# JayKickliter/Multirate.jl

Hardware: AMD Instinct MI355X
Metric: Msamples/s in (Float32, 147//160, 24*147 taps) + achieved HBM GB/s vs roofline (higher is better)
Workload: dtype f32

## Files before the change

multirate.jl_amd/csrc/mrhip_internal.h:

```cpp
#pragma once

#include <hip/hip_runtime.h>
#include <hip/hip_ext.h>

#include <cstdint>
#include <cstdlib>
#include <string>
#include <vector>

#include "multirate_hip.h"

namespace mrhip {

void set_error(const std::string &msg);
int fail(int code, const std::string &msg);

#define MRHIP_CHECK_HIP(expr)                                                                  \
    do {                                                                                       \
        hipError_t _e = (expr);                                                                \
        if (_e != hipSuccess)                                                                  \
            return ::mrhip::fail(MRHIP_ERR_HIP, std::string(#expr) + ": " + hipGetErrorString(_e)); \
    } while (0)

inline bool dtype_is_complex(int dt) { return dt == MRHIP_C64 || dt == MRHIP_C128; }
inline bool dtype_is_f64(int dt) { return dt == MRHIP_F64 || dt == MRHIP_C128; }
inline size_t dtype_scalar_size(int dt) { return dtype_is_f64(dt) ? 8 : 4; }
inline size_t dtype_size(int dt) { return dtype_scalar_size(dt) * (dtype_is_complex(dt) ? 2 : 1); }

int64_t taps2pfb(const void *h, int64_t hLen, int th, int64_t Nphi, void *out);
int64_t nextphase(int64_t phase, int64_t L, int64_t M);
int64_t outputlength_ratio(int64_t inputlength, int64_t L, int64_t M, int64_t initialPhi);
int64_t inputlength_ratio(int64_t outputlength, int64_t L, int64_t M, int64_t initialPhi);

struct CallPlan {
    int64_t n_out = 0;
    int64_t phi0 = 1, d0 = 1;
    int64_t phi_end = 1;
    int64_t d_end = 1;
    bool short_input = false;
};
CallPlan plan_rational(int kind, int64_t L, int64_t M, int64_t phiIdx, int64_t inputDeficit, int64_t xLen);

struct ArbState {
    double acc = 1.0;
    int64_t phiIdx = 1;
    double alpha = 0.0;
    int64_t xIdx = 1;
    int64_t inputDeficit = 1;
};
int64_t run_arbitrary_schedule(ArbState &st, double delta, int64_t Nphi, int64_t xLen,
                               std::vector<int32_t> *n_idx, std::vector<double> *acc_out, int mod_form = 0);
int64_t run_arbitrary_schedule_piece(ArbState &st, double delta, int64_t Nphi, int64_t xLen, int32_t *n_idx, double *acc_out,
                                     int64_t max_outputs, bool *done, int mod_form = 0);

constexpr int kSchedSeg = 64;
constexpr int kSchedGroup = 64 * kSchedSeg;
constexpr int kSchedMaxWin = 64;
constexpr int kSchedNoFail = 0x7fffffff;
constexpr int kSchedSpanSizes = 5;
constexpr int kSchedSpanBase = 64;
inline int sched_span_index(long long tile_out) { int z = 0; while (z + 1 < kSchedSpanSizes && (static_cast<long long>(kSchedSpanBase) << z) < tile_out) ++z; return z; }

struct SchedPlan {
    double delta, N, invN;
    double umin, inv_umin;
    double G, inv_G;
    double halfwin;
    int ncand, nwin;
    int pow2;
    int ok;
};
struct SchedPieceState {
    double acc;
    long long xIdx;
    double drift;
    double ksteps;
};
struct SchedStatus {
    int fail_piece;
    int done;
    long long end_k;
    double end_acc;
    long long end_xIdx;
    int max_span[kSchedSpanSizes];
    int groups_done;
    int pad[2];
    long long x_len;
    double end_drift;
    double end_ksteps;
};
struct SchedGroupEntry { double shift; int advance; int next; };
struct SchedGroupStart { double shift; long long advance; int cand; int pad; };
struct SchedPieceArgs {
    SchedPieceState *state;
    SchedStatus *status;
    double *pathT;
    int *pathW;
    SchedGroupEntry *gtab;
    SchedGroupStart *gstart;
    int *sched_n;
    double *sched_acc;
    long long k0;
    long long x_len;
    int piece, ngroups;
    int corrupt_group;
};
SchedPlan make_sched_plan(double delta, int64_t Nphi, int win_mult = 1, int win_min = 4);
struct SchedFuseArgs;
hipError_t launch_schedule_piece(const SchedPlan &c, const SchedPieceArgs &a, hipStream_t s, const SchedFuseArgs *fu = nullptr);
struct DevStream;
struct DevCall;
struct SchedBeginArgs {
    DevStream *rec;
    SchedStatus *status;
    SchedPieceState *state;
    int use_host;
    double acc; long long xIdx; double drift, ksteps;
    const DevCall *x_from;
};
struct SchedFinishArgs {
    DevStream *rec, *mirror;
    DevCall *call;
    SchedStatus *status;
    SchedPieceState *state;
    SchedPieceState *fail_state;
    int *sched_n; double *sched_acc;
    long long *count_out;
    long long k_first;
    double ks_first;
    long long pmax, est, x_len, y_capacity;
    int np;
    int serial_fallback;
};
struct SchedFuseArgs {
    int begin, finish;
    int fold_chain;
    SchedBeginArgs b;
    long long b_x_len, b_k_first;
    SchedFinishArgs f;
};
hipError_t launch_sched_begin(const SchedBeginArgs &a, long long x_len, long long k_first, hipStream_t s);
hipError_t launch_sched_finish(const SchedPlan &c, const SchedFinishArgs &a, hipStream_t s);
__host__ __device__ inline long long sched_piece_steps(double ks, long long pmax)
{
    long long P = kSchedGroup;
    while (P * 2 <= pmax && static_cast<double>(P * 2) <= 16.0 * ks) P *= 2;
    return P;
}
double sched_anchor_host(const SchedPlan &c, double acc_p, double k);

struct DevStream {
    long long phiIdx, inputDeficit;
    double acc;
    double drift, ksteps;
    long long per_pos;
    long long n_written;
    long long calls;
    long long fallback_steps;
    int error;
    int sched_fail;
};
struct DevCall {
    long long n_out;
    long long u0, d0;
    unsigned steps_per_channel, total_steps, spc_magic, pad0;
    long long per_pos, per_xbase;
    long long k_done;
    long long x_len;
};
__host__ __device__ inline unsigned step_magic(long long spc)
{
    return spc <= 1 ? 0xffffffffu : static_cast<unsigned>((1ULL << 32) / static_cast<unsigned long long>(spc));
}
struct CallPlanPOD { long long n_out, phi0, d0, phi_end, d_end; int short_input; };
__host__ __device__ inline CallPlanPOD plan_rational_pod(int kind, long long L, long long M, long long phiIdx, long long inputDeficit, long long xLen)
{
    CallPlanPOD p{0, 1, 1, 1, 1, 0};
    if (kind == MRHIP_FIR_STANDARD) { p.n_out = xLen; return p; }
    if (kind == MRHIP_FIR_INTERPOLATOR) { p.n_out = L * xLen; return p; }
    p.phi0 = kind == MRHIP_FIR_DECIMATOR ? 1 : phiIdx;
    p.d0 = inputDeficit;
    if (xLen < inputDeficit) { p.short_input = 1; p.n_out = 0; p.phi_end = phiIdx; p.d_end = inputDeficit - xLen; return p; }
    const long long a = (xLen - inputDeficit + 1) * L - p.phi0 + 1;
    p.n_out = a >= 0 ? (a + M - 1) / M : -((-a) / M);
    const long long u_end = (p.phi0 - 1) + p.n_out * M;
    p.phi_end = u_end % L + 1;
    p.d_end = p.d0 + u_end / L - xLen;
    return p;
}

struct PolyArgs {
    const void *x;
    void *y;
    const void *hist;
    void *hist_new;
    const void *taps;
    long long x_stride, y_stride;
    long long x_len;
    long long n_out;
    long long u0;
    long long d0;
    long long zero_start_below;
    int L, M, T, H;
    int nch;
    DevStream *rec;
    const DevCall *dyn;
    long long phi_end, d_end;
    const struct MultiDesc *multi;
    int multi_n;
    struct RingDev *ring_dev;
    struct RingHost *ring_host;
};

struct MultiDesc {
    const void *x;
    void *y;
    const void *hist;
    void *hist_new;
    const void *taps;
    DevStream *rec;
    long long x_stride, y_stride, x_len, n_out, u0, d0, phi_end, d_end;
    unsigned steps_per_channel, total_steps, spc_magic;
    int nch;
    int P_blk, q0;
};

constexpr int kRingDepth = 64;
constexpr int kRingTraceRows = 512, kRingTraceTiles = 32;
constexpr int kRingShards = 32;
struct RingDesc {
    unsigned long long x, y;
    long long x_stride, y_stride, x_len, n_out;
    long long u0, d0;
    unsigned long long tile_base;
    unsigned ngrabs, seq_lo;
    unsigned steps_per_channel, total_steps;
    unsigned spc_magic, flags;
    unsigned long long seq;
    unsigned long long pad[3];
};
static_assert(sizeof(RingDesc) == 128, "RingDesc is 16 quad-words");
constexpr int kRingKeyQword = 8;
struct RingHost {
    unsigned long long head;
    unsigned long long close;
    unsigned long long stopped;
    unsigned long long arrived, grid;
    unsigned long long pad[3];
    unsigned long long done[kRingDepth];
    RingDesc desc[kRingDepth];
};
struct RingDev {
    unsigned long long head;
    unsigned long long closed;
    unsigned long long idle_ticks;
    unsigned long long opts;
    unsigned long long pad[4];
    unsigned long long hist_seq[kRingDepth];
    unsigned chunk_done[kRingDepth];
    unsigned shard_done[kRingDepth][kRingShards][32];
    unsigned long long stats[24];
    unsigned long long arrived;
    unsigned long long grid;
    unsigned long long flush_req;
    unsigned long long flush_pub;
    unsigned long long flush_pad[12];
    unsigned long long flush_ent[kRingDepth][2];
    unsigned long long flush_claim[8][16];
    unsigned long long flush_done[8][16];
    unsigned long long next_ticket[8][16];
    __attribute__((aligned(128))) RingDesc desc[kRingDepth];
    unsigned long long trace[kRingTraceRows][3 * kRingTraceTiles];
};

struct ShiftFold {
    void *hist_new;
    unsigned *done;
};

struct ArbArgs {
    const void *x;
    void *y;
    const void *hist;
    const void *taps;
    const void *dtaps;
    const int *n_idx;
    const double *acc;
    long long x_stride, y_stride;
    long long x_len;
    long long n_out;
    int T, H, Nphi;
    int nch;
    const DevCall *dyn;
    ShiftFold fold;
};

struct FarrowArgs {
    const void *x;
    void *y;
    const void *hist;
    const double *pnfb;
    const int *n_idx;
    const double *acc;
    long long x_stride, y_stride;
    long long x_len;
    long long n_out;
    int T, H, polyorder;
    int tap_f32;
    int nch;
    int seam_below;
    const DevCall *dyn;
    ShiftFold fold;
};

struct HistArgs {
    const void *x;
    const void *hist_old;
    void *hist_new;
    long long x_stride;
    long long x_len;
    int H;
    int nch;
    const DevCall *dyn;
};

struct TileArgs {
    int c;
    int P;
    int J;
    int tile_len;
    int copyB_offset_bytes;
    int stage_bytes;
    int dma_rounds;
    int ablate;
    int x_aligned16;
    int by_position;
    long long tiles_per_channel;
    long long total_tiles;
};

struct PairArgs {
    int c;
    int P;
    int cM;
    int J;
    int tile_len;
    int tail;
    int dma_rounds;
    int stage_bytes;
    int ns;
    int nc;
    int x_f64, r_f64;
    int ablate;
    unsigned steps_per_channel;
    unsigned total_steps;
    unsigned steps_per_group;
    int ngroups;
    int grid_cap;
    int flags_off;
    int pad_every;
    int bank_off;
    int static_grabs;
    int rt;
    int rt_rd;
    unsigned *counters;
    unsigned spc_magic;
    int Sout, lds_step, run_chunks, q0;
    unsigned run_magic;
    long long o0;
    long long tile_in;
    long long tile_out;
    long long tiles_per_channel;
    long long total_tiles;
    unsigned long long *probe;
};

constexpr size_t kCounterBytes = 33 * 256;

struct ArbTileArgs {
    int cpl;
    int tap_pitch;
    int bank_elems;
    int x_offset_bytes;
    int max_span;
    int prefetch;
    int copyb_pad;
    int pipe;
    int row_pitch;
    int dma_slots;
    long long tile_out;
    long long tiles_per_channel;
    long long total_tiles;
    unsigned *counters;
    int run_tiles;
};

__device__ __forceinline__ void tiles_take_dyn(long long &n_out, ArbTileArgs &ta, long long &ngroups, const DevCall *dyn)
{
    ngroups = ta.tiles_per_channel > 0 ? ta.total_tiles / ta.tiles_per_channel : 1;
    if (dyn) {
        n_out = dyn->n_out;
        ta.tiles_per_channel = (n_out + ta.tile_out - 1) / ta.tile_out;
        ta.total_tiles = ta.tiles_per_channel * ngroups;
    }
}

struct LaunchEvents { hipEvent_t start = nullptr, stop = nullptr; };
extern thread_local LaunchEvents g_launch_events;

template <typename F, typename... Args>
inline void launch_kernel(F kfn, dim3 grid, dim3 block, size_t lds, hipStream_t s, Args... args)
{
    const LaunchEvents ev = g_launch_events;
    g_launch_events = LaunchEvents{};
    if (ev.start && ev.stop)
        hipExtLaunchKernelGGL(kfn, grid, block, static_cast<std::uint32_t>(lds), s, ev.start, ev.stop, 0u, args...);
    else
        hipLaunchKernelGGL(kfn, grid, block, lds, s, args...);
}

hipError_t occupancy_cached(const void *kfn, unsigned block, size_t lds, int *per_cu);

inline int env_int_read(const char *name, int dflt)
{
    const char *v = std::getenv(name);
    return v && *v ? std::atoi(v) : dflt;
}
inline bool env_dynamic()
{
    static const bool d = env_int_read("MRHIP_ENV_DYNAMIC", 0) != 0;
    return d;
}
#define MRHIP_ENV_INT(name, dflt) ([]() -> int { static const int v_ = ::mrhip::env_int_read(name, dflt); \
                                                 return ::mrhip::env_dynamic() ? ::mrhip::env_int_read(name, dflt) : v_; }())

struct TypeKey {
    bool x_f64;
    bool r_f64;
    bool complex_x;
};

hipError_t launch_poly_generic(const TypeKey &tk, bool fused, const PolyArgs &a, hipStream_t s, const char **kname);
hipError_t launch_arb_generic(const TypeKey &tk, bool fused, const ArbArgs &a, hipStream_t s, const char **kname);
hipError_t launch_farrow(const TypeKey &tk, bool fused, const FarrowArgs &a, hipStream_t s, const char **kname);
bool plan_farrow_tiled(const TypeKey &tk, const FarrowArgs &a, const int32_t *n_idx_host, const int *spans, int num_cus, ArbTileArgs *out, size_t *lds);
hipError_t launch_farrow_tiled(const TypeKey &tk, bool fused, const FarrowArgs &a, const ArbTileArgs &ta, size_t lds, hipStream_t s,
                               const char **kname, int num_cus);
hipError_t launch_shiftin(const TypeKey &tk, const HistArgs &a, hipStream_t s);
bool polyfit_rows(const double *y, int64_t n, int polyorder, double *coef);
bool plan_rational_opair(const TypeKey &tk, bool fused, const PolyArgs &a, int num_cus, PairArgs *out, dim3 *block, size_t *lds, int force_wgpc = 0);
bool plan_rational_opair_blocks(const TypeKey &tk, bool fused, const PolyArgs &a, int num_cus, PairArgs *out, dim3 *block, size_t *lds, int *nblocks);
hipError_t launch_rational_opair(bool fused, const PolyArgs &a, const PairArgs &pa, dim3 block, size_t lds, hipStream_t s,
                                 const char **kname, int num_cus, unsigned *counters);
constexpr bool opair_instantiated(bool fused, int smin, int T) { return !fused || (smin <= 1 && T % 4 == 0); }
bool plan_fir_stream(const TypeKey &tk, const PolyArgs &a, int num_cus, PairArgs *out, dim3 *block, size_t *lds);
hipError_t launch_fir_stream(bool fused, const PolyArgs &a, const PairArgs &pa, dim3 block, size_t lds, hipStream_t s,
                             const char **kname, int num_cus, unsigned *counters);
bool plan_arb_tiled(const TypeKey &tk, const ArbArgs &a, const int32_t *n_idx_host, const int *spans, int num_cus, ArbTileArgs *out, size_t *lds);
bool plan_arb_pipe(const TypeKey &tk, const ArbArgs &a, long long span256, ArbTileArgs *out, size_t *lds);
hipError_t launch_arb_pipe(const TypeKey &tk, bool fused, const ArbArgs &a, const ArbTileArgs &ta, size_t lds, hipStream_t s,
                           const char **kname, int num_cus);
struct ArbLaneArgs {
    int ring;
    int pitch8;
    int stretch;
    int chunk_max;
    int ngroups;
    int y16;
    unsigned *counters;
};
bool arb_lane_eligible(const TypeKey &tk, int T, int H, int64_t nch, double rate, int64_t x_len, int64_t x_stride, int64_t y_stride);
bool plan_arb_lane(const TypeKey &tk, const ArbArgs &a, double rate, ArbLaneArgs *out, size_t *lds);
hipError_t launch_arb_lane(bool fused, const ArbArgs &a, const ArbLaneArgs &la, size_t lds, hipStream_t s, const char **kname, int num_cus);
hipError_t launch_arb_tiled(const TypeKey &tk, bool fused, const ArbArgs &a, const ArbTileArgs &ta, size_t lds, hipStream_t s,
                            const char **kname, int num_cus);
bool plan_poly_tiled(const TypeKey &tk, const PolyArgs &a, int num_cus, ArbTileArgs *out, size_t *lds);
hipError_t launch_poly_tiled(const TypeKey &tk, bool fused, const PolyArgs &a, const ArbTileArgs &ta, size_t lds, hipStream_t s,
                             const char **kname, int num_cus);
bool plan_phase_stationary(const TypeKey &tk, const PolyArgs &a, int num_cus, TileArgs *out, dim3 *grid, dim3 *block,
                           size_t *lds);
hipError_t launch_poly_phase_stationary(const TypeKey &tk, bool fused, const PolyArgs &a, const TileArgs &ta, dim3 grid,
                                        dim3 block, size_t lds, hipStream_t s, const char **kname, int num_cus);

}
```

multirate.jl_amd/csrc/opair_kernel.inc:

```
#include <algorithm>
#include <cstdio>
#include <cstdlib>
#include <type_traits>
#include <vector>

#include "mrhip_internal.h"
#include "pair_device.h"
#include "pair_loader.h"

#pragma clang fp contract(off)

#ifndef MRHIP_OPAIR_WIDE_LONG
#define MRHIP_OPAIR_WIDE_LONG 1
#endif

namespace mrhip {
namespace {

constexpr int kOMaxThreads = 512;
constexpr int kOGroups = 32;

#define opair_env_int(name, dflt) MRHIP_ENV_INT(name, dflt)

using namespace dev;

__device__ __forceinline__ float fma_r(float a, float b, float c) { return __builtin_fmaf(a, b, c); }
__device__ __forceinline__ double fma_r(double a, double b, double c) { return __builtin_fma(a, b, c); }

template <bool FUSED, bool FIRST, bool COND, typename R>
__device__ __forceinline__ R slot_mac(R tap, R w, R acc, bool used)
{
    if constexpr (FIRST) {
        const R p = tap * w;
        if constexpr (COND) return used ? p : static_cast<R>(-0.0);
        else return p;
    } else if constexpr (FUSED) {
        const R r = fma_r(tap, w, acc);
        if constexpr (COND) return used ? r : acc;
        else return r;
    } else {
        R p = tap * w;
        if constexpr (COND) p = used ? p : static_cast<R>(-0.0);
        return acc + p;
    }
}

template <int T, bool FUSED, int NC, int SMIN, typename TXS, typename R, int MODE = 0>
#ifndef MRHIP_OPAIR_WIDE_WAVES
#define MRHIP_OPAIR_WIDE_WAVES 3
#endif
#ifndef MRHIP_RING_WAVES
#define MRHIP_RING_WAVES 4
#endif
__global__ __launch_bounds__(sizeof(R) == 8 && T > 32 ? kOMaxThreads : kOMaxThreads + 64, sizeof(R) == 8 ? (T > 32 ? 2 : MRHIP_OPAIR_WIDE_WAVES) : (MODE == 2 ? MRHIP_RING_WAVES : 3))
void rational_opair_kernel(PolyArgs a, PairArgs pa)
{
    constexpr unsigned ES = static_cast<unsigned>(sizeof(TXS)) * NC;
    constexpr unsigned OS = static_cast<unsigned>(sizeof(R)) * NC;
    constexpr int NW = static_cast<int>(ES / 4);
    static_assert(NW == 1 || NW == 2 || NW == 4, "sample size");
    using pair_t = std::conditional_t<NW == 1, v2u_t, v4u_t>;
    constexpr int SPRD = NW == 4 ? 1 : 2;
    constexpr int W = T + SMIN + 2;
    constexpr int NPR = (W + SPRD - 1) / SPRD;
    constexpr int NA = T + 1, NB = T + 2;

    extern __shared__ __attribute__((aligned(16))) unsigned char smem[];
    const unsigned lds_base = static_cast<unsigned>(reinterpret_cast<uintptr_t>(smem));
    const int tid = threadIdx.x;
    const int wave = __builtin_amdgcn_readfirstlane(tid >> 6), lane = tid & 63;
    const int ncw = (blockDim.x >> 6) - 1;
    constexpr bool RING = MODE == 2;
    if constexpr (MODE == 0) pair_take_dyn(a, pa);

    if (wave == ncw) {
        if constexpr (RING) pair_ring_loader_wave<NW, static_cast<int>(OS)>(a, pa, smem, lane);
        else pair_loader_wave<NW, MODE != 1>(a, pa, smem, lane);
        return;
    }
    if constexpr (RING) { if (blockIdx.x == 0) return; }
    volatile unsigned *const tile_flag = reinterpret_cast<volatile unsigned *>(smem + pa.flags_off);

    const int Li = static_cast<int>(a.L), Mi = static_cast<int>(a.M);
    int u0 = static_cast<int>(a.u0);
    const bool act = 2 * tid + 1 < pa.P;
    int uA = u0 + (act ? 2 * tid : 0) * Mi, uB = uA + Mi;
    int qA = uA / Li, phA = uA - qA * Li;
    int qB = uB / Li, phB = uB - qB * Li;
    int run0 = qA & ~1;
    int offA = qA - run0;
    int dB = qB - run0 - SMIN;
    R tapA[NA], tapB[NB];
    auto gather_taps = [&]() {
        const R *__restrict__ ca = static_cast<const R *>(a.taps) + static_cast<long long>(phA) * T;
        const R *__restrict__ cb = static_cast<const R *>(a.taps) + static_cast<long long>(phB) * T;
        R colA[T], colB[T];
#pragma unroll
        for (int i = 0; i < T; ++i) { colA[i] = ca[i]; colB[i] = cb[i]; }
#pragma unroll
        for (int j = 0; j < NA; ++j) {
            const R t0 = j < T ? colA[j] : R(0), t1 = j >= 1 ? colA[j - 1] : R(0);
            tapA[j] = act ? (offA == 0 ? t0 : t1) : R(0);
        }
#pragma unroll
        for (int j = 0; j < NB; ++j) {
            const R t0 = j < T ? colB[j] : R(0), t1 = (j >= 1 && j - 1 < T) ? colB[j - 1] : R(0), t2 = j >= 2 ? colB[j - 2] : R(0);
            tapB[j] = act ? (dB == 0 ? t0 : dB == 1 ? t1 : t2) : R(0);
        }
    };
    if constexpr (RING) {
#pragma unroll
        for (int j = 0; j < NA; ++j) tapA[j] = R(0);
#pragma unroll
        for (int j = 0; j < NB; ++j) tapB[j] = R(0);
        u0 = -1;
    } else if (pa.bank_off >= 0) {
        constexpr int PT = (T + 4) | 1;
        R *const bank = reinterpret_cast<R *>(smem + pa.bank_off);
        const R *__restrict__ tg = static_cast<const R *>(a.taps);
        const int ntaps = Li * T;
        for (int idx = tid; idx < ntaps; idx += ncw * 64) {
            const int col = idx / T, i = idx - col * T;
            bank[col * PT + 2 + i] = tg[idx];
        }
        asm volatile("s_waitcnt vmcnt(0) lgkmcnt(0)" ::: "memory");
        __builtin_amdgcn_s_barrier();
        const R *ba = bank + (act ? phA : 0) * PT + 2 - offA;
        const R *bb = bank + (act ? phB : 0) * PT + 2 - (act ? dB : 0);
#pragma unroll
        for (int j = 0; j < NA; ++j) tapA[j] = ba[j];
#pragma unroll
        for (int j = 0; j < NB; ++j) tapB[j] = bb[j];
#pragma unroll
        for (int j = 0; j < NA; ++j) pin(tapA[j]);
#pragma unroll
        for (int j = 0; j < NB; ++j) pin(tapB[j]);
    } else {
        const R *__restrict__ ca = static_cast<const R *>(a.taps) + static_cast<long long>(phA) * T;
        const R *__restrict__ cb = static_cast<const R *>(a.taps) + static_cast<long long>(phB) * T;
        R colA[T], colB[T];
#pragma unroll
        for (int i = 0; i < T; ++i) { colA[i] = ca[i]; colB[i] = cb[i]; }
#pragma unroll
        for (int j = 0; j < NA; ++j) {
            const R t0 = j < T ? colA[j] : R(0), t1 = j >= 1 ? colA[j - 1] : R(0);
            tapA[j] = act ? (offA == 0 ? t0 : t1) : R(0);
        }
#pragma unroll
        for (int j = 0; j < NB; ++j) {
            const R t0 = j < T ? colB[j] : R(0), t1 = (j >= 1 && j - 1 < T) ? colB[j - 1] : R(0), t2 = j >= 2 ? colB[j - 2] : R(0);
            tapB[j] = act ? (dB == 0 ? t0 : dB == 1 ? t1 : t2) : R(0);
        }
    }
    bool useA0 = offA == 0, useAT = offA == 1;
    bool useB0 = dB == 0, useB1 = dB <= 1, useBT = dB >= 1, useBT1 = dB == 2;

    const int n_out = static_cast<int>(a.n_out);
#ifdef MRHIP_OPAIR_PROBE
    unsigned long long pr_wait = 0, pr_tiles = 0;
    const unsigned long long pr_t0 = clock64(), pr_w0 = wall_clock64();
#endif
    unsigned ring_opts = 0;
    if constexpr (RING) ring_opts = static_cast<unsigned>(__builtin_amdgcn_readfirstlane(static_cast<int>(ld_sc1(&a.ring_dev->opts))));
    unsigned long long rs_bar = 0, rs_drain = 0;
    const unsigned long long rs_t0 = RING ? wall_clock64() : 0ull;
    bool pend = false;
    int p_stage = 0;
    unsigned p_slot = 0, p_shard = 0, p_cnt = 0, p_nshards = 0, p_seq_lo = 0, p_seq_hi = 0;
    for (int s = 0;; s = (s + 1 == pa.ns ? 0 : s + 1)) {
#ifdef MRHIP_OPAIR_PROBE
        const unsigned long long pr_a = clock64();
#endif
        unsigned long long rs_b0 = 0;
        if constexpr (RING) { if (ring_opts & 256u) rs_b0 = wall_clock64(); }
        __builtin_amdgcn_s_barrier();
        asm volatile("" ::: "memory");
        if constexpr (RING) { if (ring_opts & 256u) rs_bar += wall_clock64() - rs_b0; }
#ifdef MRHIP_OPAIR_PROBE
        pr_wait += clock64() - pr_a;
        ++pr_tiles;
#endif
        int J, remaining;
        R *__restrict__ yc;
        unsigned ring_flags = 0, ring_slot = 0, ring_shard = 0, ring_cnt = 0, ring_nshards = 0, ring_seq_lo = 0, ring_seq_hi = 0;
        if constexpr (RING) {
            auto word = [&](int w) -> unsigned { return static_cast<unsigned>(__builtin_amdgcn_readfirstlane(static_cast<int>(tile_flag[kRingTileWords * s + w]))); };
            const unsigned tj = word(0);
            ring_flags = word(1);
            if (pend) {
                pend = false;
                const unsigned long long rs_d0 = (ring_opts & 256u) ? wall_clock64() : 0ull;
                if (!(ring_opts & 16u)) vm_drain();
                if (ring_opts & 256u) rs_drain += wall_clock64() - rs_d0;
                if (lane == 0) {
                    unsigned *const wg_done = reinterpret_cast<unsigned *>(smem + pa.flags_off) + kRingTileWords * pa.ns;
                    const unsigned prev = __hip_atomic_fetch_add(wg_done + p_stage, 1u, __ATOMIC_RELAXED, __HIP_MEMORY_SCOPE_WORKGROUP);
                    if (prev + 1u == static_cast<unsigned>(ncw)) {
                        __hip_atomic_store(wg_done + p_stage, 0u, __ATOMIC_RELAXED, __HIP_MEMORY_SCOPE_WORKGROUP);
                        ring_grab_done(a.ring_dev, a.ring_host, p_slot, (static_cast<unsigned long long>(p_seq_hi) << 32) | p_seq_lo, p_shard, p_cnt, p_nshards);
                    }
                }
            }
            if (tj == 0u) break;
            if (ring_flags & 2u) continue;
            J = static_cast<int>(tj);
            yc = reinterpret_cast<R *>((static_cast<unsigned long long>(word(3)) << 32) | word(2));
            remaining = static_cast<int>(word(4));
            const int u0_t = static_cast<int>(word(5));
            ring_slot = word(6); ring_shard = word(7); ring_seq_lo = word(8); ring_seq_hi = word(9); ring_cnt = word(10); ring_nshards = word(11);
            if (u0_t != u0) {
                u0 = u0_t;
                uA = u0 + (act ? 2 * tid : 0) * Mi; uB = uA + Mi;
                qA = uA / Li; phA = uA - qA * Li;
                qB = uB / Li; phB = uB - qB * Li;
                run0 = qA & ~1; offA = qA - run0; dB = qB - run0 - SMIN;
                gather_taps();
                useA0 = offA == 0; useAT = offA == 1;
                useB0 = dB == 0; useB1 = dB <= 1; useBT = dB >= 1; useBT1 = dB == 2;
            }
        } else {
            const unsigned tg = static_cast<unsigned>(__builtin_amdgcn_readfirstlane(static_cast<int>(tile_flag[2 * s])));
            const unsigned tj = static_cast<unsigned>(__builtin_amdgcn_readfirstlane(static_cast<int>(tile_flag[2 * s + 1])));
            if (tj == 0u) break;
            const TileAt ta = pair_tile_at(pa, tg, tj);
            J = ta.jt;
            yc = static_cast<R *>(a.y) + (static_cast<long long>(ta.ch) * a.y_stride + static_cast<long long>(ta.st) * pa.Sout) * NC;
            remaining = n_out - ta.st * pa.Sout;
        }
        const bool full = remaining >= (J - 1) * pa.Sout + pa.P;
        unsigned lane_t;
        asm volatile("v_mbcnt_lo_u32_b32 %0, -1, 0\n\tv_mbcnt_hi_u32_b32 %0, -1, %0" : "=v"(lane_t));
        const unsigned tid_t = static_cast<unsigned>(wave) * 64u + lane_t;
        const unsigned my_out = 2u * tid_t;
        const unsigned uA_t = static_cast<unsigned>(u0) + (2u * tid_t < static_cast<unsigned>(pa.P) ? 2u * tid_t : 0u) * static_cast<unsigned>(Mi);
        const unsigned R_t = (uA_t / static_cast<unsigned>(Li)) & ~1u;
        const unsigned wbase = lds_base + static_cast<unsigned>(s) * pa.stage_bytes + (R_t - static_cast<unsigned>(pa.q0)) * ES;

        auto run_steps = [&](auto full_tag) {
            constexpr bool FULL = decltype(full_tag)::value;
            constexpr int KP = NPR < (NW == 1 ? 5 : 3) ? NPR : (NW == 1 ? 5 : 3);
            constexpr int NPRV = (NPR + KP - 1) / KP * KP;
            constexpr bool PAIRED_WAITS = KP >= 5;
            pair_t pring[KP];
            char *const ybytes = reinterpret_cast<char *>(yc);
            auto read_pair = [&](auto off_tag, unsigned addr) -> pair_t {
                constexpr int OFFP = decltype(off_tag)::value;
                if constexpr (NW == 1) return lds_read_b64<OFFP * 8>(addr);
                else return lds_read_b128<OFFP * 16>(addr);
            };
            static_for<0, KP>([&](auto I) { pring[decltype(I)::value] = read_pair(I, wbase); });
#pragma unroll 1
            for (int j = 0; j < J; ++j) {
                const int jn = j + 1 < J ? j + 1 : j;
                const unsigned wcur = wbase + static_cast<unsigned>(j) * pa.lds_step * ES;
                const unsigned wnext = wbase + static_cast<unsigned>(jn) * pa.lds_step * ES;
                R accA[NC] = {}, accB[NC] = {};
                static_for<0, NPRV>([&](auto I) {
                    constexpr int r = decltype(I)::value;
                    constexpr int slot = r % KP;
                    if constexpr (r < NPR) {
                        if constexpr (!PAIRED_WAITS) lgkm_wait<ring_younger(r, NPR, KP, 0)>(pring[slot]);
                        else if constexpr (r % 2 == 0) {
                            if constexpr (r + 1 < NPR) lgkm_wait2<ring_younger_pair(r, NPR, KP, 0)>(pring[slot], pring[(r + 1) % KP]);
                            else lgkm_wait<ring_younger(r, NPR, KP, 0)>(pring[slot]);
                        }
                        R wv[2][NC];
                        if constexpr (NW == 4) {
                            wv[0][0] = __hiloint2double(static_cast<int>(pring[slot].y), static_cast<int>(pring[slot].x));
                            wv[0][1] = __hiloint2double(static_cast<int>(pring[slot].w), static_cast<int>(pring[slot].z));
                        } else if constexpr (sizeof(TXS) == 8) {
                            wv[0][0] = __hiloint2double(static_cast<int>(pring[slot].y), static_cast<int>(pring[slot].x));
                            wv[1][0] = __hiloint2double(static_cast<int>(pring[slot].w), static_cast<int>(pring[slot].z));
                        } else if constexpr (NC == 1) {
                            wv[0][0] = static_cast<R>(__uint_as_float(pring[slot].x)); wv[1][0] = static_cast<R>(__uint_as_float(pring[slot].y));
                        } else {
                            wv[0][0] = static_cast<R>(__uint_as_float(pring[slot].x)); wv[0][1] = static_cast<R>(__uint_as_float(pring[slot].y));
                            wv[1][0] = static_cast<R>(__uint_as_float(pring[slot].z)); wv[1][1] = static_cast<R>(__uint_as_float(pring[slot].w));
                        }
                        static_for<0, SPRD>([&](auto H) {
                            constexpr int js = SPRD * r + decltype(H)::value;
                            constexpr int jb = js - SMIN;
                            constexpr bool a_lo = js < 1, a_hi = js > T - 1;
                            constexpr bool b_lo = jb < 2, b_hi = jb > T - 1;
#pragma unroll
                            for (int cc = 0; cc < NC; ++cc) {
                                const R w = wv[decltype(H)::value][cc];
                                if constexpr (js < NA) {
                                    const bool used = (a_lo ? useA0 : true) && (a_hi ? useAT : true);
                                    accA[cc] = slot_mac<FUSED, js == 0, a_lo || a_hi, R>(tapA[js], w, accA[cc], used);
                                }
                                if constexpr (jb >= 0 && jb < NB) {
                                    const bool used = (b_lo ? (jb == 0 ? useB0 : useB1) : true) && (b_hi ? (jb == T ? useBT : useBT1) : true);
                                    accB[cc] = slot_mac<FUSED, jb == 0, b_lo || b_hi, R>(tapB[jb], w, accB[cc], used);
                                }
                            }
                        });
#pragma unroll
                        for (int cc = 0; cc < NC; ++cc) { pin(accA[cc]); pin(accB[cc]); }
                    }
                    if constexpr (r + KP < NPR) pring[slot] = read_pair(std::integral_constant<int, r + KP>{}, wcur);
                    else if constexpr (r + KP >= NPRV) pring[slot] = read_pair(std::integral_constant<int, r + KP - NPRV>{}, wnext);
                });
                {
                    const unsigned kj = static_cast<unsigned>(j) * static_cast<unsigned>(pa.Sout);
                    char *const dst = ybytes + (kj + my_out) * OS;
                    R v[2 * NC];
#pragma unroll
                    for (int cc = 0; cc < NC; ++cc) { v[cc] = accA[cc]; v[NC + cc] = accB[cc]; }
                    auto put2 = [&]() { if constexpr (RING) { if (ring_nshards >> 31) { store_wt<2 * OS>(dst, v); return; } } __builtin_memcpy(dst, v, 2 * OS); };
                    auto put1 = [&]() { if constexpr (RING) { if (ring_nshards >> 31) { store_wt<OS>(dst, v); return; } } __builtin_memcpy(dst, v, OS); };
                    bool covered = false;
                    if constexpr (RING && 2 * OS == 8) {
                        if (!(ring_nshards >> 31)) {
                            covered = true;
                            const unsigned lim_x = FULL ? static_cast<unsigned>(pa.P) : (static_cast<unsigned>(remaining) > kj ? umin(static_cast<unsigned>(remaining) - kj, static_cast<unsigned>(pa.P)) : 0u);
                            if (my_out + 1 < lim_x) __builtin_memcpy(dst, v, 2 * OS);
                            else if (my_out < lim_x) __builtin_memcpy(dst, v, OS);
                        } else if (ring_opts & 8u) {
                            unsigned q[4];
                            q[0] = __float_as_uint(v[0]); q[1] = __float_as_uint(v[1]);
                            q[2] = static_cast<unsigned>(__builtin_amdgcn_mov_dpp(static_cast<int>(q[0]), 0xF5, 0xF, 0xF, false));
                            q[3] = static_cast<unsigned>(__builtin_amdgcn_mov_dpp(static_cast<int>(q[1]), 0xF5, 0xF, 0xF, false));
                            const unsigned lim_x = FULL ? static_cast<unsigned>(pa.P) : (static_cast<unsigned>(remaining) > kj ? umin(static_cast<unsigned>(remaining) - kj, static_cast<unsigned>(pa.P)) : 0u);
                            const bool even = (lane_t & 1u) == 0u;
                            if (even && my_out + 3 < lim_x) {
                                if (ring_opts & 2048u) {
                                    v4u_t qq; __builtin_memcpy(&qq, q, 16);
                                    asm volatile("global_store_dwordx4 %0, %1, off sc0 sc1" ::"v"(dst), "v"(qq) : "memory");
                                } else store_wt<16>(dst, q);
                                covered = true;
                            }
                            else if (!even && my_out + 1 < lim_x) covered = true;
                        }
                    }
                    if (!covered) {
                    if constexpr (FULL) {
                        if (my_out + 1 < static_cast<unsigned>(pa.P)) put2();
                    } else {
                        const unsigned rem_j = static_cast<unsigned>(remaining) > kj ? static_cast<unsigned>(remaining) - kj : 0u;
                        const unsigned lim = rem_j < static_cast<unsigned>(pa.P) ? rem_j : static_cast<unsigned>(pa.P);
                        if (my_out + 1 < lim) put2();
                        else if (my_out < lim) put1();
                    }
                    }
                }
            }
            lgkm_wait<0>(pring[0]);
            static_for<0, KP>([&](auto I) { pin(pring[decltype(I)::value]); });
        };
        if (full) run_steps(std::true_type{});
        else run_steps(std::false_type{});
        if constexpr (RING) {
            if (ring_flags & 1u) {
                pend = true; p_stage = s;
                p_slot = ring_slot; p_shard = ring_shard; p_cnt = ring_cnt; p_nshards = ring_nshards; p_seq_lo = ring_seq_lo; p_seq_hi = ring_seq_hi;
                if (ring_opts & 2u) {
                    pend = false;
                    vm_drain();
                    if (lane == 0) {
                        unsigned *const wg_done = reinterpret_cast<unsigned *>(smem + pa.flags_off) + kRingTileWords * pa.ns;
                        const unsigned prev = __hip_atomic_fetch_add(wg_done + p_stage, 1u, __ATOMIC_RELAXED, __HIP_MEMORY_SCOPE_WORKGROUP);
                        if (prev + 1u == static_cast<unsigned>(ncw)) {
                            __hip_atomic_store(wg_done + p_stage, 0u, __ATOMIC_RELAXED, __HIP_MEMORY_SCOPE_WORKGROUP);
                            ring_grab_done(a.ring_dev, a.ring_host, p_slot, (static_cast<unsigned long long>(p_seq_hi) << 32) | p_seq_lo, p_shard, p_cnt, p_nshards);
                        }
                    }
                }
            }
        }
    }
    if constexpr (RING) {
        if ((ring_opts & 256u) && lane == 0) {
            atomicAdd(&a.ring_dev->stats[0], wall_clock64() - rs_t0);
            atomicAdd(&a.ring_dev->stats[1], rs_bar);
            atomicAdd(&a.ring_dev->stats[2], rs_drain);
            atomicAdd(&a.ring_dev->stats[3], 1ull);
        }
    }
#ifdef MRHIP_OPAIR_PROBE
    if (pa.probe && lane == 0) {
        unsigned long long *r = pa.probe + (static_cast<unsigned long long>(blockIdx.x) * 8u + static_cast<unsigned>(wave)) * 4u;
        const unsigned hw = __builtin_amdgcn_s_getreg(0xF804), xcc = __builtin_amdgcn_s_getreg(0xF814);
        r[0] = hw | (static_cast<unsigned long long>(xcc) << 32);
        r[1] = clock64() - pr_t0; r[2] = pr_wait; r[3] = pr_tiles | ((wall_clock64() - pr_w0) << 32);
    }
#endif
}

#ifdef MRHIP_OPAIR_PROBE
inline unsigned long long *opair_probe_buf(long long g)
{
    static unsigned long long *buf = nullptr;
    static long long cap = 0;
    if (!std::getenv("MRHIP_PROBE_OUT")) return nullptr;
    if (g > cap) { if (buf) (void)hipFree(buf); (void)hipMalloc(&buf, static_cast<size_t>(g) * 8 * 4 * 8); cap = g; }
    (void)hipMemset(buf, 0, static_cast<size_t>(g) * 8 * 4 * 8);
    (void)hipDeviceSynchronize();
    return buf;
}
inline void opair_probe_dump(unsigned long long *buf, long long g, hipStream_t s)
{
    if (!buf) return;
    (void)hipStreamSynchronize(s);
    std::vector<unsigned long long> h(static_cast<size_t>(g) * 8 * 4);
    (void)hipMemcpy(h.data(), buf, h.size() * 8, hipMemcpyDeviceToHost);
    if (FILE *f = std::fopen(std::getenv("MRHIP_PROBE_OUT"), "wb")) { std::fwrite(h.data(), 8, h.size(), f); std::fclose(f); }
}
#define MRHIP_PROBE_PRE(g) pa.probe = opair_probe_buf(g);
#define MRHIP_PROBE_POST(g) opair_probe_dump(pa.probe, g, s);
#else
#define MRHIP_PROBE_PRE(g)
#define MRHIP_PROBE_POST(g)
#endif

template <typename TXS, typename R>
constexpr bool opair_plain_instantiated(bool fused, int nc, int smin, int T)
{
    return !fused && smin <= 1 && (T == 24 || T == 32) && (nc >= 1) && sizeof(TXS) >= 4 && sizeof(R) >= 4;
}
template <bool FUSED, int NC, int SMIN, typename TXS, typename R>
hipError_t launch_opair_T(int T, dim3 block, size_t lds, hipStream_t s, const PolyArgs &a, PairArgs pa, int num_cus)
{
#define MRHIP_CASE(TT)                                                                              \
    case TT: if constexpr (opair_instantiated(FUSED, SMIN, TT)) {                                   \
        auto kfn = rational_opair_kernel<TT, FUSED, NC, SMIN, TXS, R>;                                       \
        if constexpr (opair_plain_instantiated<TXS, R>(FUSED, NC, SMIN, TT)) {                      \
            if (a.ring_dev) kfn = rational_opair_kernel<TT, FUSED, NC, SMIN, TXS, R, 2>;            \
                                                                                             \
            else if (!a.dyn && !a.multi && opair_env_int("MRHIP_OPAIR_PLAIN", 1))                                                           \
                kfn = a.n_out * a.nch >= (1LL << 22) ? rational_opair_kernel<TT, FUSED, NC, SMIN, TXS, R, 1> : rational_opair_kernel<TT, FUSED, NC, SMIN, TXS, R, 3>; \
        } else if (a.ring_dev) return hipErrorNotSupported;                                         \
        int per_cu = 0;                                                                             \
        hipError_t eo = occupancy_cached(reinterpret_cast<const void *>(kfn), block.x, lds, &per_cu); \
        if (eo != hipSuccess) return eo;                                                            \
        if (per_cu < 1) per_cu = 1;                                                                 \
        {    \
            const long long tiles = (static_cast<long long>(pa.total_steps) + pa.J - 1) / pa.J;     \
            if (block.x == 6 * 64 && per_cu > 3 && tiles > 3LL * num_cus * per_cu) per_cu = 3;      \
        }                                                                                           \
        const int bpc = opair_env_int("MRHIP_OPAIR_BPC", 0);                                 \
        if (bpc > 0) per_cu = bpc;                                                                  \
        long long g = static_cast<long long>(num_cus) * per_cu;                                     \
        if (g > static_cast<long long>(pa.total_steps)) g = pa.total_steps;                         \
        if (g < 1) g = 1;                                                                           \
        if (a.ring_dev) { g = static_cast<long long>(num_cus) * per_cu;    \
            if (pa.grid_cap > 1 && g > pa.grid_cap) g = pa.grid_cap; }                                  \
        pa.ngroups = static_cast<int>(g < kOGroups ? g : kOGroups);                                 \
        if (!a.ring_dev) pa.steps_per_group = static_cast<unsigned>((pa.total_steps + pa.ngroups - 1) / pa.ngroups);    \
        pa.static_grabs = (static_cast<long long>(pa.total_steps) + pa.J - 1) / pa.J <= 3 * g;      \
        if (a.multi) {    \
            long long w = static_cast<long long>(num_cus) * per_cu / a.multi_n;                     \
            const long long tiles = (static_cast<long long>(pa.total_steps) + pa.J - 1) / pa.J;     \
            if (w > tiles) w = tiles;                                                               \
            if (w < 1) w = 1;                                                                       \
            g = w * a.multi_n;                                                                      \
            pa.ngroups = a.multi_n;                                                                 \
            pa.static_grabs = 1;                                                                    \
        }                                                                                           \
        static int dbg = opair_env_int("MRHIP_DEBUG", 0);                                           \
        if (dbg == 1) {                                                                             \
            dbg = 0;                                                                                \
            hipFuncAttributes fa;                                                                   \
            (void)hipFuncGetAttributes(&fa, reinterpret_cast<const void *>(kfn));                   \
            std::fprintf(stderr, "[mrhip] rational_opair T=%d smin=%d in=%zuB arith=%zuB grid=%lld block=%u lds=%zu occ/CU=%d regs=%d c=%d P=%d cM=%d J=%d ns=%d\n", \
                         TT, SMIN, sizeof(TXS) * NC, sizeof(R), g, block.x, lds, per_cu, fa.numRegs, pa.c, pa.P, pa.cM, pa.J, pa.ns); \
        }                                                                                           \
        MRHIP_PROBE_PRE(g)                                                                          \
        launch_kernel(kfn, dim3(static_cast<unsigned>(g)), block, lds, s, a, pa);                   \
        MRHIP_PROBE_POST(g)                                                                         \
        return hipGetLastError();                                                                   \
    } else break;
#ifdef MRHIP_OPAIR_LONG
    switch (T) {
#ifdef MRHIP_PS_FAST_BUILD
        MRHIP_CASE(56) MRHIP_CASE(64)
#else
        MRHIP_CASE(49) MRHIP_CASE(50) MRHIP_CASE(51) MRHIP_CASE(52) MRHIP_CASE(53) MRHIP_CASE(54) MRHIP_CASE(55) MRHIP_CASE(56)
        MRHIP_CASE(57) MRHIP_CASE(58) MRHIP_CASE(59) MRHIP_CASE(60) MRHIP_CASE(61) MRHIP_CASE(62) MRHIP_CASE(63) MRHIP_CASE(64)
#endif
    default: break;
    }
#else
    switch (T) {
#ifdef MRHIP_PS_FAST_BUILD
        MRHIP_CASE(24)
#else
        MRHIP_CASE(1) MRHIP_CASE(2) MRHIP_CASE(3) MRHIP_CASE(4) MRHIP_CASE(5) MRHIP_CASE(6) MRHIP_CASE(7) MRHIP_CASE(8)
        MRHIP_CASE(9) MRHIP_CASE(10) MRHIP_CASE(11) MRHIP_CASE(12) MRHIP_CASE(13) MRHIP_CASE(14) MRHIP_CASE(15) MRHIP_CASE(16)
        MRHIP_CASE(17) MRHIP_CASE(18) MRHIP_CASE(19) MRHIP_CASE(20) MRHIP_CASE(21) MRHIP_CASE(22) MRHIP_CASE(23) MRHIP_CASE(24)
        MRHIP_CASE(25) MRHIP_CASE(26) MRHIP_CASE(27) MRHIP_CASE(28) MRHIP_CASE(29) MRHIP_CASE(30) MRHIP_CASE(31) MRHIP_CASE(32)
#endif
    default: break;
    }
    if constexpr ((sizeof(R) == 4 || (NC == 1 && MRHIP_OPAIR_WIDE_LONG)) && SMIN <= 1) {
        switch (T) {
#ifndef MRHIP_PS_FAST_BUILD
        MRHIP_CASE(33) MRHIP_CASE(34) MRHIP_CASE(35) MRHIP_CASE(36) MRHIP_CASE(37) MRHIP_CASE(38) MRHIP_CASE(39) MRHIP_CASE(40)
        MRHIP_CASE(41) MRHIP_CASE(42) MRHIP_CASE(43) MRHIP_CASE(44) MRHIP_CASE(45) MRHIP_CASE(46) MRHIP_CASE(47) MRHIP_CASE(48)
#else
        MRHIP_CASE(36) MRHIP_CASE(48)
#endif
        default: break;
        }
    }
#endif
    return hipErrorInvalidValue;
#undef MRHIP_CASE
}

}
}
```

Before: 653,000.

## Sort output pairs into uniform-class waves to drop conditional MAC slots

For f32 T=24 plain-mode launches, each compute wave classifies its output pairs by phase alignment (offset of A and B within the input run). Using ballots, it then remaps thread-to-pair assignments so whole waves hold a single class. Those waves run a specialized inner loop with compile-time tap offsets, which skips the conditional select slots and extra LDS pair reads. This adds setup cost (two classification passes over all waves at kernel start) and extra code instantiations, which may raise register pressure.

```diff
diff --git a/multirate.jl_amd/csrc/mrhip_internal.h b/multirate.jl_amd/csrc/mrhip_internal.h
--- a/multirate.jl_amd/csrc/mrhip_internal.h
+++ b/multirate.jl_amd/csrc/mrhip_internal.h
@@ -363,6 +363,7 @@
     int static_grabs;
     int rt;
     int rt_rd;
+    int sorted;
     unsigned *counters;
     unsigned spc_magic;
     int Sout, lds_step, run_chunks, q0;
diff --git a/multirate.jl_amd/csrc/opair_kernel.inc b/multirate.jl_amd/csrc/opair_kernel.inc
--- a/multirate.jl_amd/csrc/opair_kernel.inc
+++ b/multirate.jl_amd/csrc/opair_kernel.inc
@@ -62,7 +62,6 @@
     using pair_t = std::conditional_t<NW == 1, v2u_t, v4u_t>;
     constexpr int SPRD = NW == 4 ? 1 : 2;
     constexpr int W = T + SMIN + 2;
-    constexpr int NPR = (W + SPRD - 1) / SPRD;
     constexpr int NA = T + 1, NB = T + 2;
 
     extern __shared__ __attribute__((aligned(16))) unsigned char smem[];
@@ -83,8 +82,65 @@
 
     const int Li = static_cast<int>(a.L), Mi = static_cast<int>(a.M);
     int u0 = static_cast<int>(a.u0);
-    const bool act = 2 * tid + 1 < pa.P;
-    int uA = u0 + (act ? 2 * tid : 0) * Mi, uB = uA + Mi;
+    constexpr bool SORTABLE = (MODE == 1 || MODE == 3) && !FUSED && sizeof(R) == 4 && T == 24 && SMIN <= 1;
+    constexpr int DD = SMIN == 0 ? 1 : 0;
+    int pidx = tid;
+    int wcls = 2;
+    if constexpr (SORTABLE) {
+        if (pa.sorted) {
+            const float invL = __builtin_amdgcn_rcpf(static_cast<float>(Li));
+            auto quot = [&](int u) -> int {
+                int q = static_cast<int>(static_cast<float>(u) * invL);
+                const int r = u - q * Li;
+                q += r >= Li ? 1 : 0;
+                q -= r < 0 ? 1 : 0;
+                return q;
+            };
+            auto pair_class = [&](int t) -> int {
+                const bool has = 2 * t + 1 < pa.P;
+                const int ua = u0 + (has ? 2 * t : 0) * Mi;
+                const int qa = quot(ua), qb = quot(ua + Mi);
+                const int oa = qa & 1, db = qb - (qa & ~1) - SMIN;
+                return has && db == oa + DD ? oa : 2;
+            };
+            int c0 = 0, c1 = 0;
+            for (int w = 0; w < ncw; ++w) {
+                const int k = pair_class(w * 64 + lane);
+                c0 += __popcll(__ballot(k == 0));
+                c1 += __popcll(__ballot(k == 1));
+            }
+            const int n0 = c0 >> 6, n1 = c1 >> 6;
+            if (2 * (n0 + n1) >= ncw) {
+                wcls = wave < n0 ? 0 : wave < n0 + n1 ? 1 : 2;
+                const int want = (wave - (wcls == 0 ? 0 : wcls == 1 ? n0 : n0 + n1)) * 64 + lane;
+                int r0 = 0, r1 = 0, rt = 0;
+                for (int w = 0; w < ncw; ++w) {
+                    const int k = pair_class(w * 64 + lane);
+                    const unsigned long long m0 = __ballot(k == 0), m1 = __ballot(k == 1);
+                    const int below0 = static_cast<int>(__builtin_amdgcn_mbcnt_hi(static_cast<unsigned>(m0 >> 32), __builtin_amdgcn_mbcnt_lo(static_cast<unsigned>(m0), 0u)));
+                    const int below1 = static_cast<int>(__builtin_amdgcn_mbcnt_hi(static_cast<unsigned>(m1 >> 32), __builtin_amdgcn_mbcnt_lo(static_cast<unsigned>(m1), 0u)));
+                    const unsigned long long p0 = __ballot(k == 0 && r0 + below0 < 64 * n0);
+                    const unsigned long long p1 = __ballot(k == 1 && r1 + below1 < 64 * n1);
+                    const unsigned long long mt = wcls == 0 ? p0 : wcls == 1 ? p1 : ~(p0 | p1);
+                    const int cnt = __popcll(mt);
+                    const int d = want - rt;
+                    if (d >= 0 && d < cnt) {
+                        unsigned pos = 0, kk = static_cast<unsigned>(d);
+#pragma unroll
+                        for (unsigned sft = 32; sft >= 1; sft >>= 1) {
+                            const unsigned cc = static_cast<unsigned>(__popcll((mt >> pos) & ((1ull << sft) - 1ull)));
+                            if (kk >= cc) { kk -= cc; pos += sft; }
+                        }
+                        pidx = w * 64 + static_cast<int>(pos);
+                    }
+                    rt += cnt; r0 += __popcll(m0); r1 += __popcll(m1);
+                }
+                wcls = __builtin_amdgcn_readfirstlane(wcls);
+            }
+        }
+    }
+    const bool act = 2 * pidx + 1 < pa.P;
+    int uA = u0 + (act ? 2 * pidx : 0) * Mi, uB = uA + Mi;
     int qA = uA / Li, phA = uA - qA * Li;
     int qB = uB / Li, phB = uB - qB * Li;
     int run0 = qA & ~1;
@@ -230,14 +286,20 @@
         const bool full = remaining >= (J - 1) * pa.Sout + pa.P;
         unsigned lane_t;
         asm volatile("v_mbcnt_lo_u32_b32 %0, -1, 0\n\tv_mbcnt_hi_u32_b32 %0, -1, %0" : "=v"(lane_t));
-        const unsigned tid_t = static_cast<unsigned>(wave) * 64u + lane_t;
+        unsigned tid_t = static_cast<unsigned>(wave) * 64u + lane_t;
+        if constexpr (SORTABLE) asm volatile("v_mov_b32 %0, %1" : "=v"(tid_t) : "v"(pidx));
         const unsigned my_out = 2u * tid_t;
         const unsigned uA_t = static_cast<unsigned>(u0) + (2u * tid_t < static_cast<unsigned>(pa.P) ? 2u * tid_t : 0u) * static_cast<unsigned>(Mi);
         const unsigned R_t = (uA_t / static_cast<unsigned>(Li)) & ~1u;
         const unsigned wbase = lds_base + static_cast<unsigned>(s) * pa.stage_bytes + (R_t - static_cast<unsigned>(pa.q0)) * ES;
 
-        auto run_steps = [&](auto full_tag) {
+        auto run_steps = [&](auto full_tag, auto cls_tag) {
             constexpr bool FULL = decltype(full_tag)::value;
+            constexpr int CLS = decltype(cls_tag)::value;
+            constexpr bool PURE = CLS >= 0;
+            constexpr int OFFA = PURE ? CLS : 0, DB = PURE ? CLS + DD : 0;
+            constexpr int LAST = OFFA + T - 1 > SMIN + DB + T - 1 ? OFFA + T - 1 : SMIN + DB + T - 1;
+            constexpr int NPR = PURE ? LAST / SPRD + 1 : (W + SPRD - 1) / SPRD;
             constexpr int KP = NPR < (NW == 1 ? 5 : 3) ? NPR : (NW == 1 ? 5 : 3);
             constexpr int NPRV = (NPR + KP - 1) / KP * KP;
             constexpr bool PAIRED_WAITS = KP >= 5;
@@ -285,6 +347,10 @@
 #pragma unroll
                             for (int cc = 0; cc < NC; ++cc) {
                                 const R w = wv[decltype(H)::value][cc];
+                                if constexpr (PURE) {
+                                    if constexpr (js >= OFFA && js <= OFFA + T - 1) accA[cc] = slot_mac<FUSED, js == OFFA, false, R>(tapA[js], w, accA[cc], true);
+                                    if constexpr (jb >= DB && jb <= DB + T - 1) accB[cc] = slot_mac<FUSED, jb == DB, false, R>(tapB[jb], w, accB[cc], true);
+                                } else {
                                 if constexpr (js < NA) {
                                     const bool used = (a_lo ? useA0 : true) && (a_hi ? useAT : true);
                                     accA[cc] = slot_mac<FUSED, js == 0, a_lo || a_hi, R>(tapA[js], w, accA[cc], used);
@@ -292,6 +358,7 @@
                                 if constexpr (jb >= 0 && jb < NB) {
                                     const bool used = (b_lo ? (jb == 0 ? useB0 : useB1) : true) && (b_hi ? (jb == T ? useBT : useBT1) : true);
                                     accB[cc] = slot_mac<FUSED, jb == 0, b_lo || b_hi, R>(tapB[jb], w, accB[cc], used);
+                                }
                                 }
                             }
                         });
@@ -348,8 +415,15 @@
             lgkm_wait<0>(pring[0]);
             static_for<0, KP>([&](auto I) { pin(pring[decltype(I)::value]); });
         };
-        if (full) run_steps(std::true_type{});
-        else run_steps(std::false_type{});
+        auto run_class = [&](auto cls_tag) {
+            if (full) run_steps(std::true_type{}, cls_tag);
+            else run_steps(std::false_type{}, cls_tag);
+        };
+        if constexpr (SORTABLE) {
+            if (wcls == 0) run_class(std::integral_constant<int, 0>{});
+            else if (wcls == 1) run_class(std::integral_constant<int, 1>{});
+            else run_class(std::integral_constant<int, -1>{});
+        } else run_class(std::integral_constant<int, -1>{});
         if constexpr (RING) {
             if (ring_flags & 1u) {
                 pend = true; p_stage = s;
@@ -427,8 +501,11 @@
         if constexpr (opair_plain_instantiated<TXS, R>(FUSED, NC, SMIN, TT)) {                      \
             if (a.ring_dev) kfn = rational_opair_kernel<TT, FUSED, NC, SMIN, TXS, R, 2>;            \
                                                                                              \
-            else if (!a.dyn && !a.multi && opair_env_int("MRHIP_OPAIR_PLAIN", 1))                                                           \
+            else if (!a.dyn && !a.multi && opair_env_int("MRHIP_OPAIR_PLAIN", 1)) {                                                         \
                 kfn = a.n_out * a.nch >= (1LL << 22) ? rational_opair_kernel<TT, FUSED, NC, SMIN, TXS, R, 1> : rational_opair_kernel<TT, FUSED, NC, SMIN, TXS, R, 3>; \
+                 \
+                pa.sorted = pa.run_chunks == 0 && pa.Sout == pa.P && opair_env_int("MRHIP_OPAIR_SORTED", 1) != 0;                           \
+            }                                                                                                                               \
         } else if (a.ring_dev) return hipErrorNotSupported;                                         \
         int per_cu = 0;                                                                             \
         hipError_t eo = occupancy_cached(reinterpret_cast<const void *>(kfn), block.x, lds, &per_cu); \
```

New measurement: 616,900. -5.5%, worse.
